# yanqinJiang/Animate3D

Measured on AMD Instinct MI355X. Metric: UNet denoise-steps/sec, 4view×16frame×512² MV-VDM @1/2/4/8 GPU, higher is better.
Workload: dtype bf16; 1 GPU; BASELINE config 2: 4 views x 16 frames x 512^2 px (64x64 latent), CFG-doubled batch V=8 videos, one MVUNetMotionModel.forward per step, SD1.5 MV-VDM UNet 1.53 B params, seeded synthetic weights; parallelism=single GPU

## Files before the change

animate3d_amd/csrc/gemm_common.h:

```cpp
#pragma once
#include "common.h"

struct GemmParams {
  const uint16_t* X; int64_t ldx;
  const uint16_t* W; int64_t ldw;
  const float* bias;
  const uint16_t* rowbias; int64_t rb_div;
  const uint16_t* R; int64_t ldr;
  uint16_t* Y; int64_t ldy;
  int64_t M, N, K;
  float alpha, beta;
  int vec16;
  int out_f32;
  int abl;
  int B, H, Wd, Cin, Ho, Wo, stride, up, He, We;
  int64_t tiles_n, tiles_m;
  int ksplit, nk_item;
  float* ws; int64_t ws_bytes;
  const uint16_t* X2; int64_t ldx2; int64_t K1;
  int direct;
};

constexpr int EPI_LINEAR = 0, EPI_GEGLU = 1;

static inline int a3d_gemm_kernel_of(int flags) { return flags & A3D_GEMM_KERNEL_MASK; }
static inline int a3d_gemm_reserved_cus_of(int flags) { return flags & A3D_GEMM_RESERVED_CUS_MASK; }

A3D_DEV float epi_scale(float v, float alpha) { return __fmul_rn(v, alpha); }
A3D_DEV float epi_axpy(float v, float beta, float r) { return __fmaf_rn(beta, r, v); }

A3D_DEV float gelu_erf(float gte) {
  const float x = fabsf(gte) * 0.70710678118654752f;
  const float t = __builtin_amdgcn_rcpf(fmaf(0.3275911f, x, 1.0f));
  float poly = fmaf(1.061405429f, t, -1.453152027f);
  poly = fmaf(poly, t, 1.421413741f);
  poly = fmaf(poly, t, -0.284496736f);
  poly = fmaf(poly, t, 0.254829592f);
  poly *= t;
  const float e = __builtin_amdgcn_exp2f(-x * x * 1.4426950408889634f);
  const float erfx = fmaf(-poly, e, 1.0f);
  const float hg = __fmul_rn(0.5f, gte);
  return __fmaf_rn(fabsf(hg), erfx, hg);
}

A3D_DEV f32x2_t splat2(float v) { return f32x2_t{v, v}; }
A3D_DEV f32x2_t gelu_erf2(f32x2_t g) {
  const f32x2_t x = __builtin_elementwise_abs(g) * 0.70710678118654752f;
  const f32x2_t den = __builtin_elementwise_fma(splat2(0.3275911f), x, splat2(1.0f));
  const f32x2_t t = {__builtin_amdgcn_rcpf(den[0]), __builtin_amdgcn_rcpf(den[1])};
  f32x2_t poly = __builtin_elementwise_fma(splat2(1.061405429f), t, splat2(-1.453152027f));
  poly = __builtin_elementwise_fma(poly, t, splat2(1.421413741f));
  poly = __builtin_elementwise_fma(poly, t, splat2(-0.284496736f));
  poly = __builtin_elementwise_fma(poly, t, splat2(0.254829592f));
  poly = poly * t;
  const f32x2_t a = (-x) * x * 1.4426950408889634f;
  const f32x2_t e = {__builtin_amdgcn_exp2f(a[0]), __builtin_amdgcn_exp2f(a[1])};
  const f32x2_t erfx = __builtin_elementwise_fma(-poly, e, splat2(1.0f));
  const f32x2_t hg = g * 0.5f;
  return __builtin_elementwise_fma(__builtin_elementwise_abs(hg), erfx, hg);
}
A3D_DEV void geglu8(const float (&hv)[8], const float (&gv)[8], const float (&bh)[8], const float (&bg)[8], float (&y)[8]) {
#pragma unroll
  for (int e = 0; e < 4; ++e) {
    const f32x2_t gg = f32x2_t{gv[2 * e], gv[2 * e + 1]} + f32x2_t{bg[2 * e], bg[2 * e + 1]};
    const f32x2_t hh = f32x2_t{hv[2 * e], hv[2 * e + 1]} + f32x2_t{bh[2 * e], bh[2 * e + 1]};
    const f32x2_t yy = hh * gelu_erf2(gg);
    y[2 * e] = yy[0]; y[2 * e + 1] = yy[1];
  }
}

static __device__ u32x4_t g_zero_page[4];

A3D_DEV uint32_t lds_addr(const void* p) {
  return (uint32_t)(uintptr_t)(__attribute__((address_space(3))) const void*)p;
}
A3D_DEV void glds16_v(const void* gsrc, uint32_t lds_dst) {
  unsigned keep;
  asm volatile("s_mov_b32 %0, m0\n\ts_mov_b32 m0, %2\n\ts_nop 0\n\tglobal_load_lds_dwordx4 %1, off\n\ts_mov_b32 m0, %0"
               : "=&s"(keep) : "v"(gsrc), "s"(__builtin_amdgcn_readfirstlane(lds_dst)) : "memory");
}
A3D_DEV void glds16_s(uint32_t voff, const void* sbase, uint32_t lds_dst) {
  unsigned keep;
  asm volatile("s_mov_b32 %0, m0\n\ts_mov_b32 m0, %3\n\ts_nop 0\n\tglobal_load_lds_dwordx4 %1, %2\n\ts_mov_b32 m0, %0"
               : "=&s"(keep) : "v"(voff), "s"(sbase), "s"(__builtin_amdgcn_readfirstlane(lds_dst)) : "memory");
}
A3D_DEV const uint16_t* scalar_ptr(const uint16_t* ptr) {
  const uint64_t a = (uint64_t)(uintptr_t)ptr;
  return (const uint16_t*)(uintptr_t)(((uint64_t)(uint32_t)__builtin_amdgcn_readfirstlane((int)(a >> 32)) << 32) |
                                      (uint32_t)__builtin_amdgcn_readfirstlane((int)(uint32_t)a));
}
A3D_DEV u32x4_t lds_vload128(const void* p) {
  return *(const volatile __attribute__((address_space(3))) u32x4_t*)(uintptr_t)lds_addr(p);
}
A3D_DEV u32x2_t lds_vload64(const void* p) {
  return *(const volatile __attribute__((address_space(3))) u32x2_t*)(uintptr_t)lds_addr(p);
}
A3D_DEV void wave_lds_fence() {
  __builtin_amdgcn_fence(__ATOMIC_RELEASE, "wavefront");
  __builtin_amdgcn_wave_barrier();
  __builtin_amdgcn_fence(__ATOMIC_ACQUIRE, "wavefront");
}

template <int EPI, int NB, bool RES>
A3D_DEV void persist_epilogue(const GemmParams& p, f32x16_t (&acc)[NB][2], float* const stg, const float* const bias_lds,
                              const uint16_t* const rowbias_lds, const int64_t m0, const int64_t n0, const int wm, const int wblk,
                              const int wblk_last, const int lane) {
  const int l31 = lane & 31, g = lane >> 5;
  constexpr int SROW = 68;
  constexpr int NP = (NB + 1) / 2;
  u32x4_t rres[RES ? 2 : 1][RES ? 4 : 1];
  auto pass_cols = [&](int ps) { return (2 * ps + 1 < NB) ? 64 : 32; };
  auto pass_col0 = [&](int ps) { return ((2 * ps + 1 < NB) ? wblk + 2 * ps : wblk_last) * 32; };
  auto load_res = [&](int pi, int slot) {
    if constexpr (RES) {
      const int tm = pi / NP, ps = pi % NP;
      const int64_t mbase = m0 + wm * 64 + tm * 32;
      const int64_t nbase = n0 + pass_col0(ps);
      if (pass_cols(ps) == 64) {
#pragma unroll
        for (int j = 0; j < 4; ++j) {
          const int64_t m = mbase + 8 * j + (lane >> 3);
          rres[slot][j] = *reinterpret_cast<const u32x4_t*>(p.R + m * p.ldr + nbase + 8 * (lane & 7));
        }
      } else {
#pragma unroll
        for (int j = 0; j < 2; ++j) {
          const int64_t m = mbase + 16 * j + (lane >> 2);
          rres[slot][j] = *reinterpret_cast<const u32x4_t*>(p.R + m * p.ldr + nbase + 8 * (lane & 3));
        }
      }
    }
  };
  if constexpr (RES) load_res(0, 0);
  if constexpr (EPI == EPI_GEGLU || !RES) {
    constexpr int RS = (EPI == EPI_GEGLU) ? 64 : 128;
    char* const stg16 = reinterpret_cast<char*>(stg);
    const int wsw = (EPI == EPI_GEGLU) ? ((l31 >> 1) & 3) : (l31 & 7);
    const int whalf = 8 * (g ^ ((l31 >> 3) & 1));
    auto unswap = [](u32x4_t o, int row) {
      const bool sw = row & 8;
      u32x4_t r;
      r[0] = sw ? o[2] : o[0]; r[1] = sw ? o[3] : o[1]; r[2] = sw ? o[0] : o[2]; r[3] = sw ? o[1] : o[3];
      return r;
    };
    constexpr int BUF2 = 32 * RS;
#pragma unroll
    for (int pi = 0; pi < 2 * NP; ++pi) {
      const int tm = pi / NP, ps = pi % NP;
      const int ncol = pass_cols(ps);
      const int64_t mbase = m0 + wm * 64 + tm * 32;
      const int64_t nbase = n0 + pass_col0(ps);
      char* const sb = stg16 + (pi & 1) * BUF2;
      if constexpr (EPI == EPI_GEGLU) {
        u32x4_t bq[2][4];
        auto fetch = [&](int q2, int slot) __attribute__((always_inline)) {
#pragma unroll
          for (int h = 0; h < 2; ++h) {
            const int c0 = 8 * (2 * q2 + h) + 4 * g;
            bq[slot][2 * h] = lds_vload128(bias_lds + pass_col0(ps) + c0);
            bq[slot][2 * h + 1] = lds_vload128(bias_lds + pass_col0(ps) + 32 + c0);
          }
        };
        fetch(0, 0);
#pragma unroll
        for (int q2 = 0; q2 < 2; ++q2) {
          if (q2 + 1 < 2) fetch(q2 + 1, (q2 + 1) & 1);
          __builtin_amdgcn_sched_barrier(0);
          float hv[8], gv[8], bh[8], bg[8], y[8];
#pragma unroll
          for (int h = 0; h < 2; ++h) {
            const u32x4_t b0 = bq[q2 & 1][2 * h], b1 = bq[q2 & 1][2 * h + 1];
#pragma unroll
            for (int j = 0; j < 4; ++j) { bh[4 * h + j] = __uint_as_float(b0[j]); bg[4 * h + j] = __uint_as_float(b1[j]); }
#pragma unroll
            for (int j = 0; j < 4; ++j) { hv[4 * h + j] = acc[2 * ps][tm][4 * (2 * q2 + h) + j]; gv[4 * h + j] = acc[2 * ps + 1][tm][4 * (2 * q2 + h) + j]; }
          }
          geglu8(hv, gv, bh, bg, y);
#pragma unroll
          for (int h = 0; h < 2; ++h) {
            u32x2_t o;
            o[0] = pack16(y[4 * h], y[4 * h + 1]);
            o[1] = pack16(y[4 * h + 2], y[4 * h + 3]);
            *reinterpret_cast<u32x2_t*>(sb + l31 * RS + 16 * ((2 * q2 + h) ^ wsw) + whalf) = o;
          }
        }
        wave_lds_fence();
        const int cc = lane & 3;
        const int64_t oc = nbase / 2 + 8 * cc;
        u32x4_t ob[2];
#pragma unroll
        for (int j = 0; j < 2; ++j) {
          const int row = 16 * j + (lane >> 2);
          ob[j] = *reinterpret_cast<const u32x4_t*>(sb + row * RS + 16 * (cc ^ ((row >> 1) & 3)));
        }
#pragma unroll
        for (int j = 0; j < 2; ++j) {
          const int row = 16 * j + (lane >> 2);
          const int64_t m = mbase + row;
          const u32x4_t o = unswap(ob[j], row);
#ifdef A3D_ABLATIONS
          if (p.abl & 2) { asm volatile("" :: "v"(o[0]), "v"(o[1]), "v"(o[2]), "v"(o[3])); continue; }
          *reinterpret_cast<u32x4_t*>(p.Y + ((p.abl & 1) ? (m & 255) : m) * p.ldy + oc) = o;
#else
          *reinterpret_cast<u32x4_t*>(p.Y + m * p.ldy + oc) = o;
#endif
        }
      } else {
        constexpr int NQ = 8;
        const int nq = (2 * ps + 1 < NB) ? 8 : 4;
        u32x4_t bq[3];
        u32x2_t tq[3];
        auto fetch = [&](int idx, int slot) __attribute__((always_inline)) {
          const int c0 = (idx >> 2) * 32 + 8 * (idx & 3) + 4 * g;
          bq[slot] = lds_vload128(bias_lds + pass_col0(ps) + c0);
          tq[slot] = lds_vload64(rowbias_lds + pass_col0(ps) + c0);
        };
        auto quads = [&](auto with_c) __attribute__((always_inline)) {
          constexpr bool WITH = decltype(with_c)::value;
          if constexpr (WITH) { fetch(0, 0); fetch(1, 1); }
#pragma unroll
          for (int idx = 0; idx < NQ; ++idx) {
            if (idx >= nq) continue;
            const int tl = idx >> 2, q = idx & 3;
            const int tn = 2 * ps + tl;
            if constexpr (WITH) {
              if (idx + 2 < nq) fetch(idx + 2, (idx + 2) % 3);
              __builtin_amdgcn_sched_barrier(0);
            }
            float v[4] = {acc[tn][tm][4 * q], acc[tn][tm][4 * q + 1], acc[tn][tm][4 * q + 2], acc[tn][tm][4 * q + 3]};
            if constexpr (WITH) {
              const u32x4_t b = bq[idx % 3];
              v[0] += __uint_as_float(b[0]); v[1] += __uint_as_float(b[1]); v[2] += __uint_as_float(b[2]); v[3] += __uint_as_float(b[3]);
              const u32x2_t tb = tq[idx % 3];
              v[0] += lo16(tb[0]); v[1] += hi16(tb[0]); v[2] += lo16(tb[1]); v[3] += hi16(tb[1]);
            }
#pragma unroll
            for (int e = 0; e < 4; ++e) v[e] = epi_scale(v[e], p.alpha);
            u32x2_t o;
            o[0] = pack16(v[0], v[1]);
            o[1] = pack16(v[2], v[3]);
            *reinterpret_cast<u32x2_t*>(sb + l31 * RS + 16 * ((4 * tl + q) ^ wsw) + whalf) = o;
            if constexpr (WITH) __builtin_amdgcn_sched_barrier(0);
          }
        };
        if (p.bias || p.rowbias) quads(std::true_type{});
        else quads(std::false_type{});
        wave_lds_fence();
        const int lpr = ncol / 8;
        const int cc = lane & (lpr - 1);
        u32x4_t ob[4];
#pragma unroll
        for (int j = 0; j < 4; ++j) {
          if (j * (64 / lpr) >= 32) continue;
          const int row = (64 / lpr) * j + lane / lpr;
          ob[j] = *reinterpret_cast<const u32x4_t*>(sb + row * RS + 16 * (cc ^ (row & 7)));
        }
#pragma unroll
        for (int j = 0; j < 4; ++j) {
          if (j * (64 / lpr) >= 32) continue;
          const int row = (64 / lpr) * j + lane / lpr;
          const int64_t m = mbase + row;
          const u32x4_t o = unswap(ob[j], row);
#ifdef A3D_ABLATIONS
          if (p.abl & 2) { asm volatile("" :: "v"(o[0]), "v"(o[1]), "v"(o[2]), "v"(o[3])); continue; }
          *reinterpret_cast<u32x4_t*>(p.Y + ((p.abl & 1) ? (m & 255) : m) * p.ldy + nbase + 8 * cc) = o;
#else
          *reinterpret_cast<u32x4_t*>(p.Y + m * p.ldy + nbase + 8 * cc) = o;
#endif
        }
      }
    }
    return;
  }
#pragma unroll
  for (int pi = 0; pi < 2 * NP; ++pi) {
    const int tm = pi / NP, ps = pi % NP;
    const int ncol = pass_cols(ps);
    if constexpr (RES) { if (pi + 1 < 2 * NP) load_res(pi + 1, (pi + 1) & 1); }
#pragma unroll
    for (int tl = 0; tl < 2; ++tl) {
      const int tn = 2 * ps + tl;
      if (tn < NB) {
#pragma unroll
        for (int q = 0; q < 4; ++q) {
          float4 v;
          v.x = acc[tn][tm][4 * q]; v.y = acc[tn][tm][4 * q + 1]; v.z = acc[tn][tm][4 * q + 2]; v.w = acc[tn][tm][4 * q + 3];
          *reinterpret_cast<float4*>(stg + l31 * SROW + tl * 32 + 8 * q + 4 * g) = v;
        }
      }
    }
    wave_lds_fence();
    const int64_t mbase = m0 + wm * 64 + tm * 32;
    const int64_t nbase = n0 + pass_col0(ps);

    if constexpr (EPI == EPI_GEGLU) {
      const int cc = lane & 3;
      const int64_t oc = nbase / 2 + 8 * cc;
      float bh[8], bg[8];
      {
        const float* bl = bias_lds + (pass_col0(ps) + 8 * cc);
#pragma unroll
        for (int e = 0; e < 8; ++e) { bh[e] = bl[e]; bg[e] = bl[32 + e]; }
      }
#pragma unroll
      for (int j = 0; j < 2; ++j) {
        const int row = 16 * j + (lane >> 2);
        const int64_t m = mbase + row;
        const float4 h0 = *reinterpret_cast<const float4*>(stg + row * SROW + 8 * cc);
        const float4 h1 = *reinterpret_cast<const float4*>(stg + row * SROW + 8 * cc + 4);
        const float4 g0 = *reinterpret_cast<const float4*>(stg + row * SROW + 32 + 8 * cc);
        const float4 g1 = *reinterpret_cast<const float4*>(stg + row * SROW + 32 + 8 * cc + 4);
        const float hv[8] = {h0.x, h0.y, h0.z, h0.w, h1.x, h1.y, h1.z, h1.w};
        const float gv[8] = {g0.x, g0.y, g0.z, g0.w, g1.x, g1.y, g1.z, g1.w};
        float y[8];
        geglu8(hv, gv, bh, bg, y);
        u32x4_t o;
#pragma unroll
        for (int e = 0; e < 4; ++e) o[e] = pack16(y[2 * e], y[2 * e + 1]);
#ifdef A3D_ABLATIONS
        if (p.abl & 2) { asm volatile("" :: "v"(o[0]), "v"(o[1]), "v"(o[2]), "v"(o[3])); continue; }
        *reinterpret_cast<u32x4_t*>(p.Y + ((p.abl & 1) ? (m & 255) : m) * p.ldy + oc) = o;
#else
        *reinterpret_cast<u32x4_t*>(p.Y + m * p.ldy + oc) = o;
#endif
      }
    } else {
      const int lpr = ncol / 8;
      const int cc = lane & (lpr - 1);
      const int64_t n = nbase + 8 * cc;
      const int ncl = pass_col0(ps) + 8 * cc;
      float bv[8];
#pragma unroll
      for (int e = 0; e < 8; ++e) bv[e] = bias_lds[ncl + e];
      const u32x4_t tb = *reinterpret_cast<const u32x4_t*>(rowbias_lds + ncl);
#pragma unroll
      for (int j = 0; j < 4; ++j) {
        if (j * (64 / lpr) >= 32) continue;
        const int row = (64 / lpr) * j + lane / lpr;
        const int64_t m = mbase + row;
        const float4 a0 = *reinterpret_cast<const float4*>(stg + row * SROW + 8 * cc);
        const float4 a1 = *reinterpret_cast<const float4*>(stg + row * SROW + 8 * cc + 4);
        float v[8] = {a0.x, a0.y, a0.z, a0.w, a1.x, a1.y, a1.z, a1.w};
#pragma unroll
        for (int e = 0; e < 8; ++e) v[e] += bv[e];
#pragma unroll
        for (int e = 0; e < 4; ++e) { v[2 * e] += lo16(tb[e]); v[2 * e + 1] += hi16(tb[e]); }
#pragma unroll
        for (int e = 0; e < 8; ++e) v[e] = epi_scale(v[e], p.alpha);
        if constexpr (RES) {
          const u32x4_t tr = rres[pi & 1][j];
#pragma unroll
          for (int e = 0; e < 4; ++e) { v[2 * e] = epi_axpy(v[2 * e], p.beta, lo16(tr[e])); v[2 * e + 1] = epi_axpy(v[2 * e + 1], p.beta, hi16(tr[e])); }
        }
        u32x4_t o;
#pragma unroll
        for (int e = 0; e < 4; ++e) o[e] = pack16(v[2 * e], v[2 * e + 1]);
#ifdef A3D_ABLATIONS
        if (p.abl & 2) { asm volatile("" :: "v"(o[0]), "v"(o[1]), "v"(o[2]), "v"(o[3])); continue; }
        *reinterpret_cast<u32x4_t*>(p.Y + ((p.abl & 1) ? (m & 255) : m) * p.ldy + n) = o;
#else
        *reinterpret_cast<u32x4_t*>(p.Y + m * p.ldy + n) = o;
#endif
      }
    }
    wave_lds_fence();
  }
}

template <int NB, bool RES>
A3D_DEV void direct_epilogue(const GemmParams& p, f32x16_t (&acc)[NB][2], const float* const bias_lds, const uint16_t* const rowbias_lds,
                             const int64_t m0, const int64_t n0, const int wm, const int wblk, const int wblk_last, const int lane) {
  const int l31 = lane & 31, g = lane >> 5;
  const bool with = p.bias || p.rowbias;
#pragma unroll
  for (int tm = 0; tm < 2; ++tm) {
    const int64_t m = m0 + wm * 64 + tm * 32 + l31;
    uint16_t* const yrow = p.Y + m * p.ldy + n0;
    u32x4_t rr[RES ? NB : 1][2];
    if constexpr (RES) {
      const uint16_t* const rrow = p.R + m * p.ldr + n0;
#pragma unroll
      for (int tn = 0; tn < NB; ++tn) {
        const int col = (tn < NB - 1 ? wblk + tn : wblk_last) * 32 + 16 * g;
        rr[tn][0] = *reinterpret_cast<const u32x4_t*>(rrow + col);
        rr[tn][1] = *reinterpret_cast<const u32x4_t*>(rrow + col + 8);
      }
    }
#pragma unroll
    for (int tn = 0; tn < NB; ++tn) {
      const int col = (tn < NB - 1 ? wblk + tn : wblk_last) * 32 + 16 * g;
      float v[16];
#pragma unroll
      for (int r = 0; r < 16; ++r) v[r] = acc[tn][tm][r];
      if (with) {
#pragma unroll
        for (int q = 0; q < 4; ++q) {
          const u32x4_t b = lds_vload128(bias_lds + col + 4 * q);
#pragma unroll
          for (int e = 0; e < 4; ++e) v[4 * q + e] += __uint_as_float(b[e]);
        }
#pragma unroll
        for (int h = 0; h < 2; ++h) {
          const u32x4_t tb = lds_vload128(rowbias_lds + col + 8 * h);
#pragma unroll
          for (int e = 0; e < 4; ++e) { v[8 * h + 2 * e] += lo16(tb[e]); v[8 * h + 2 * e + 1] += hi16(tb[e]); }
        }
      }
#pragma unroll
      for (int r = 0; r < 16; ++r) v[r] = epi_scale(v[r], p.alpha);
      if constexpr (RES) {
#pragma unroll
        for (int h = 0; h < 2; ++h)
#pragma unroll
          for (int e = 0; e < 4; ++e) {
            v[8 * h + 2 * e] = epi_axpy(v[8 * h + 2 * e], p.beta, lo16(rr[tn][h][e]));
            v[8 * h + 2 * e + 1] = epi_axpy(v[8 * h + 2 * e + 1], p.beta, hi16(rr[tn][h][e]));
          }
      }
#pragma unroll
      for (int h = 0; h < 2; ++h) {
        u32x4_t o;
#pragma unroll
        for (int e = 0; e < 4; ++e) o[e] = pack16(v[8 * h + 2 * e], v[8 * h + 2 * e + 1]);
        *reinterpret_cast<u32x4_t*>(yrow + col + 8 * h) = o;
      }
    }
  }
}

__attribute__((visibility("hidden"))) int A3D_FN(a3d_launch_gemm_pp)(int conv, int epi, int nb, hipStream_t stream, const GemmParams& p, int cus);
__attribute__((visibility("hidden"))) int A3D_FN(a3d_launch_gemm_ring)(int nb, hipStream_t stream, const GemmParams& p, int cus);
```

animate3d_amd/csrc/gemm_conv.hip:

```cpp
#include "gemm_common.h"

namespace {

constexpr int BM = 128, BN = 128;
template <int BKT> struct TileCfg {
  static constexpr int LROW = BKT + 8;
  static constexpr int TILE_ELEMS = 128 * LROW;
  static constexpr int STAGE_BYTES = 2 * 2 * TILE_ELEMS * 2;
  static constexpr int EPI_BYTES = 4 * 32 * 68 * 4;
  static constexpr int SMEM_BYTES = STAGE_BYTES > EPI_BYTES ? STAGE_BYTES : EPI_BYTES;
  static constexpr int CPR = BKT / 8;
  static constexpr int RPT = 256 / CPR;
  static constexpr int NPASS = 128 / RPT;
};



template <int CONV, int EPI, int BKT, bool RES>
__global__ __launch_bounds__(256, (BKT == 64 ? 2 : 3)) void gemm_kernel(const GemmParams p) {
  using TC = TileCfg<BKT>;
  constexpr int LROW = TC::LROW, TILE_ELEMS = TC::TILE_ELEMS, NPASS = TC::NPASS, RPT = TC::RPT, BK = BKT;
  extern __shared__ __attribute__((aligned(16))) uint16_t smem[];
  const int tid = threadIdx.x;
  const int lane = tid & 63, wid = tid >> 6;
  const int wm = wid >> 1, wn = wid & 1;
  const int l31 = lane & 31, g = lane >> 5;

  const int64_t nblk = p.tiles_n * p.tiles_m;
  const int64_t lid = xcd_remap(blockIdx.x, nblk);
  const int64_t tile_n = lid % p.tiles_n, tile_m = lid / p.tiles_n;
  const int64_t m0 = tile_m * BM, n0 = tile_n * BN;

  const int kc = tid % TC::CPR;
  const int srow = tid / TC::CPR;

  const uint16_t* a_ptr[NPASS];
  int a_b[CONV == 2 ? NPASS : 1], a_y[CONV == 2 ? NPASS : 1], a_x[CONV == 2 ? NPASS : 1];
  bool a_ok[NPASS];
  int a_mask[NPASS];
#pragma unroll
  for (int i = 0; i < NPASS; ++i) {
    int64_t m = m0 + srow + RPT * i;
    a_ok[i] = m < p.M;
    if (m >= p.M) m = p.M - 1;
    if constexpr (CONV != 0) {
      const int hw = p.Ho * p.Wo;
      const int b = (int)(m / hw);
      const int rem = (int)(m - (int64_t)b * hw);
      const int oy = rem / p.Wo, ox = rem - oy * p.Wo;
      if constexpr (CONV == 2) {
        a_b[i] = b; a_y[i] = oy; a_x[i] = ox;
        a_ptr[i] = nullptr; a_mask[i] = 0;
      } else {
        const int y0 = oy * p.stride - 1, x0 = ox * p.stride - 1;
        a_ptr[i] = p.X + (((int64_t)b * p.H + y0) * p.Wd + x0) * p.Cin + kc * 8;
        int mask = 0;
#pragma unroll
        for (int t = 0; t < 9; ++t) {
          const int yy = y0 + t / 3, xx = x0 + t % 3;
          if (a_ok[i] && yy >= 0 && yy < p.H && xx >= 0 && xx < p.Wd) mask |= 1 << t;
        }
        a_mask[i] = mask;
      }
    } else {
      a_ptr[i] = p.X + m * p.ldx + kc * 8;
      a_mask[i] = 0;
    }
  }
  const uint16_t* w_ptr[NPASS];
#pragma unroll
  for (int i = 0; i < NPASS; ++i) {
    int64_t n = n0 + srow + RPT * i;
    if (n >= p.N) n = p.N - 1;
    w_ptr[i] = p.W + n * p.ldw + kc * 8;
  }

  struct RegTile { u32x4_t a[NPASS], w[NPASS]; };
  RegTile rt0, rt1;
  auto load_tile = [&](int64_t k0, RegTile& rt) {
    u32x4_t (&ra)[NPASS] = rt.a; u32x4_t (&rw)[NPASS] = rt.w;
    if constexpr (CONV != 0) {
      {
        const int kt64 = (int)(k0 >> 6);
        const int c64 = kt64 / 9, t = kt64 - 9 * c64;
        k0 = (int64_t)t * p.Cin + c64 * 64 + (k0 & 63);
      }
      const int tap = (int)(k0 / p.Cin);
      const int ci0 = (int)(k0 - (int64_t)tap * p.Cin);
      const int ky = tap / 3, kx = tap - ky * 3;
      if constexpr (CONV == 1) {
        const int64_t toff = ((int64_t)ky * p.Wd + kx) * p.Cin + ci0;
#pragma unroll
        for (int i = 0; i < NPASS; ++i) {
          if ((a_mask[i] >> tap) & 1) ra[i] = *reinterpret_cast<const u32x4_t*>(a_ptr[i] + toff);
          else ra[i] = u32x4_t{0u, 0u, 0u, 0u};
        }
      } else {
        const int He = p.He, We = p.We;
#pragma unroll
        for (int i = 0; i < NPASS; ++i) {
          const int yy = a_y[i] + ky - 1, xx = a_x[i] + kx - 1;
          const bool ok = a_ok[i] && yy >= 0 && yy < He && xx >= 0 && xx < We;
          if (ok) {
            const uint16_t* src = p.X + (((int64_t)a_b[i] * p.H + (yy >> 1)) * p.Wd + (xx >> 1)) * p.Cin + ci0 + kc * 8;
            ra[i] = *reinterpret_cast<const u32x4_t*>(src);
          } else {
            ra[i] = u32x4_t{0u, 0u, 0u, 0u};
          }
        }
      }
    } else {
#pragma unroll
      for (int i = 0; i < NPASS; ++i) ra[i] = *reinterpret_cast<const u32x4_t*>(a_ptr[i] + k0);
    }
#pragma unroll
    for (int i = 0; i < NPASS; ++i) rw[i] = *reinterpret_cast<const u32x4_t*>(w_ptr[i] + k0);
  };
  auto store_tile = [&](int buf, const RegTile& rt) {
    const u32x4_t (&ra)[NPASS] = rt.a; const u32x4_t (&rw)[NPASS] = rt.w;
    uint16_t* As = smem + (buf * 2 + 0) * TILE_ELEMS;
    uint16_t* Ws = smem + (buf * 2 + 1) * TILE_ELEMS;
#pragma unroll
    for (int i = 0; i < NPASS; ++i) {
      *reinterpret_cast<u32x4_t*>(As + (srow + RPT * i) * LROW + kc * 8) = ra[i];
      *reinterpret_cast<u32x4_t*>(Ws + (srow + RPT * i) * LROW + kc * 8) = rw[i];
    }
  };

  f32x16_t acc[2][2];
#pragma unroll
  for (int a = 0; a < 2; ++a)
#pragma unroll
    for (int b = 0; b < 2; ++b)
#pragma unroll
      for (int r = 0; r < 16; ++r) acc[a][b][r] = 0.f;

  u32x4_t rres[RES ? 4 : 1];
  const int ecc = lane & 7;
  const int64_t en = n0 + wn * 64 + 8 * ecc;
  const bool epf = RES && (EPI == EPI_LINEAR) && p.R != nullptr && p.vec16 && en + 8 <= p.N;
  auto prefetch_residual = [&](int tm) {
    if constexpr (RES) {
#pragma unroll
      for (int j = 0; j < 4; ++j) {
        int64_t m = m0 + wm * 64 + tm * 32 + 8 * j + (lane >> 3);
        if (m >= p.M) m = p.M - 1;
        rres[j] = *reinterpret_cast<const u32x4_t*>(p.R + m * p.ldr + en);
      }
    }
  };

  const int64_t nk = p.K / BK;
  auto compute = [&](int cur) {
    const uint16_t* As = smem + (cur * 2 + 0) * TILE_ELEMS;
    const uint16_t* Ws = smem + (cur * 2 + 1) * TILE_ELEMS;
    u32x4_t fw[2][2], fa[2][2];
    auto load_frags = [&](int slot, int ks) {
#pragma unroll
      for (int t = 0; t < 2; ++t) {
        fw[slot][t] = *reinterpret_cast<const u32x4_t*>(Ws + (wn * 64 + t * 32 + l31) * LROW + ks * 16 + g * 8);
        fa[slot][t] = *reinterpret_cast<const u32x4_t*>(As + (wm * 64 + t * 32 + l31) * LROW + ks * 16 + g * 8);
      }
    };
    load_frags(0, 0);
#pragma unroll
    for (int ks = 0; ks < BK / 16; ++ks) {
      if (ks + 1 < BK / 16) load_frags((ks + 1) & 1, ks + 1);
#pragma unroll
      for (int tn = 0; tn < 2; ++tn)
#pragma unroll
        for (int tm = 0; tm < 2; ++tm) acc[tn][tm] = mfma32(fw[ks & 1][tn], fa[ks & 1][tm], acc[tn][tm]);
    }
  };

  load_tile(0, rt0);
  store_tile(0, rt0);
  if (nk > 1) load_tile(1 * BK, rt0);
  if (nk > 2) load_tile(2 * BK, rt1);
  __syncthreads();
  for (int64_t kt = 0;;) {
    if (kt + 1 >= nk && epf) prefetch_residual(0);
    compute(0);
    if (kt + 1 < nk) store_tile(1, rt0);
    if (kt + 3 < nk) load_tile((kt + 3) * BK, rt0);
    __syncthreads();
    if (++kt >= nk) break;
    if (kt + 1 >= nk && epf) prefetch_residual(0);
    compute(1);
    if (kt + 1 < nk) store_tile(0, rt1);
    if (kt + 3 < nk) load_tile((kt + 3) * BK, rt1);
    __syncthreads();
    if (++kt >= nk) break;
  }

  constexpr int SROW = 68;
  float* const stg = reinterpret_cast<float*>(smem) + wid * (32 * SROW);
#pragma unroll
  for (int tm = 0; tm < 2; ++tm) {
  if (tm == 1) __syncthreads();
#pragma unroll
  for (int tn = 0; tn < 2; ++tn)
#pragma unroll
    for (int q = 0; q < 4; ++q) {
      float4 v;
      v.x = acc[tn][tm][4 * q]; v.y = acc[tn][tm][4 * q + 1]; v.z = acc[tn][tm][4 * q + 2]; v.w = acc[tn][tm][4 * q + 3];
      *reinterpret_cast<float4*>(stg + l31 * SROW + tn * 32 + 8 * q + 4 * g) = v;
    }
  __syncthreads();
  const int64_t mbase = m0 + wm * 64 + tm * 32;

  if constexpr (EPI == EPI_GEGLU) {
    const int cc = lane & 3;
    const int64_t nh = n0 + wn * 64 + 8 * cc;
    const int64_t oc = (n0 + wn * 64) / 2 + 8 * cc;
    if (nh + 32 < p.N + 0 && oc + 8 <= p.N / 2) {
      float bh[8], bg[8];
#pragma unroll
      for (int e = 0; e < 8; ++e) { bh[e] = p.bias ? p.bias[nh + e] : 0.f; bg[e] = p.bias ? p.bias[nh + 32 + e] : 0.f; }
#pragma unroll
      for (int j = 0; j < 2; ++j) {
        const int row = 16 * j + (lane >> 2);
        const int64_t m = mbase + row;
        if (m >= p.M) continue;
        const float4 h0 = *reinterpret_cast<const float4*>(stg + row * SROW + 8 * cc);
        const float4 h1 = *reinterpret_cast<const float4*>(stg + row * SROW + 8 * cc + 4);
        const float4 g0 = *reinterpret_cast<const float4*>(stg + row * SROW + 32 + 8 * cc);
        const float4 g1 = *reinterpret_cast<const float4*>(stg + row * SROW + 32 + 8 * cc + 4);
        const float hv[8] = {h0.x, h0.y, h0.z, h0.w, h1.x, h1.y, h1.z, h1.w};
        const float gv[8] = {g0.x, g0.y, g0.z, g0.w, g1.x, g1.y, g1.z, g1.w};
        float y[8];
        geglu8(hv, gv, bh, bg, y);
        u32x4_t o;
#pragma unroll
        for (int e = 0; e < 4; ++e) o[e] = pack16(y[2 * e], y[2 * e + 1]);
        *reinterpret_cast<u32x4_t*>(p.Y + m * p.ldy + oc) = o;
      }
    }
  } else {
    const int cc = lane & 7;
    const int64_t n = n0 + wn * 64 + 8 * cc;
    if (n < p.N) {
      const bool full = (n + 8 <= p.N) && p.vec16;
      float bv[8];
#pragma unroll
      for (int e = 0; e < 8; ++e) bv[e] = (p.bias && n + e < p.N) ? p.bias[n + e] : 0.f;
#pragma unroll
      for (int j = 0; j < 4; ++j) {
        const int row = 8 * j + (lane >> 3);
        const int64_t m = mbase + row;
        if (m >= p.M) continue;
        const float4 a0 = *reinterpret_cast<const float4*>(stg + row * SROW + 8 * cc);
        const float4 a1 = *reinterpret_cast<const float4*>(stg + row * SROW + 8 * cc + 4);
        float v[8] = {a0.x, a0.y, a0.z, a0.w, a1.x, a1.y, a1.z, a1.w};
#pragma unroll
        for (int e = 0; e < 8; ++e) v[e] += bv[e];
        const uint16_t* rb = p.rowbias ? p.rowbias + (m / p.rb_div) * p.N + n : nullptr;
        const uint16_t* rr = p.R ? p.R + m * p.ldr + n : nullptr;
        uint16_t* yy = p.Y + m * p.ldy + n;
        if (full) {
          if (rb) {
            const u32x4_t t = *reinterpret_cast<const u32x4_t*>(rb);
#pragma unroll
            for (int e = 0; e < 4; ++e) { v[2 * e] += lo16(t[e]); v[2 * e + 1] += hi16(t[e]); }
          }
#pragma unroll
          for (int e = 0; e < 8; ++e) v[e] = epi_scale(v[e], p.alpha);
          if constexpr (RES) {
            if (rr) {
              const u32x4_t t = rres[j];
#pragma unroll
              for (int e = 0; e < 4; ++e) { v[2 * e] = epi_axpy(v[2 * e], p.beta, lo16(t[e])); v[2 * e + 1] = epi_axpy(v[2 * e + 1], p.beta, hi16(t[e])); }
            }
          }
          if (p.out_f32) {
            float* yf = reinterpret_cast<float*>(p.Y) + m * p.ldy + n;
            *reinterpret_cast<float4*>(yf) = float4{v[0], v[1], v[2], v[3]};
            *reinterpret_cast<float4*>(yf + 4) = float4{v[4], v[5], v[6], v[7]};
          } else {
            u32x4_t o;
#pragma unroll
            for (int e = 0; e < 4; ++e) o[e] = pack16(v[2 * e], v[2 * e + 1]);
            *reinterpret_cast<u32x4_t*>(yy) = o;
          }
        } else {
#pragma unroll
          for (int hh = 0; hh < 2; ++hh) {
            if (n + 4 * hh + 4 > p.N) continue;
            float w[4] = {v[4 * hh], v[4 * hh + 1], v[4 * hh + 2], v[4 * hh + 3]};
            if (rb) {
              const u32x2_t t = *reinterpret_cast<const u32x2_t*>(rb + 4 * hh);
              w[0] += lo16(t[0]); w[1] += hi16(t[0]); w[2] += lo16(t[1]); w[3] += hi16(t[1]);
            }
#pragma unroll
            for (int e = 0; e < 4; ++e) w[e] = epi_scale(w[e], p.alpha);
            if (rr) {
              const u32x2_t t = *reinterpret_cast<const u32x2_t*>(rr + 4 * hh);
              w[0] = epi_axpy(w[0], p.beta, lo16(t[0])); w[1] = epi_axpy(w[1], p.beta, hi16(t[0]));
              w[2] = epi_axpy(w[2], p.beta, lo16(t[1])); w[3] = epi_axpy(w[3], p.beta, hi16(t[1]));
            }
            u32x2_t o;
            o[0] = pack16(w[0], w[1]);
            o[1] = pack16(w[2], w[3]);
            *reinterpret_cast<u32x2_t*>(yy + 4 * hh) = o;
          }
        }
      }
    }
  }
  if (tm == 0 && epf) prefetch_residual(1);
  }
}


constexpr int PBM = 256;
constexpr int PERSIST_MIN_FILL = 50;
struct PPPlan { int nb, S, cus; int64_t tiles_m, tiles_n; };
constexpr int SPLITK_MAX = 16;
#ifndef A3D_EXP_SPLITK_MINK
#define A3D_EXP_SPLITK_MINK 9
#endif
template <int CONV, int EPI>
bool plan_persist(const GemmParams& p, int flags, bool allow_split, PPPlan& out) {
  if (a3d_gemm_kernel_of(flags) == A3D_GEMM_TILE128 || p.out_f32) return false;
  static int cus_of[64] = {0};
  const int dev = a3d_current_device();
  if (cus_of[dev] == 0) {
    int n = 0;
    if (hipDeviceGetAttribute(&n, hipDeviceAttributeMultiprocessorCount, dev) != hipSuccess) return false;
    cus_of[dev] = n > 0 ? n : 256;
  }
  const int reserved = a3d_gemm_reserved_cus_of(flags);
  const int cus = cus_of[dev] - reserved > 32 ? cus_of[dev] - reserved : 32;
  if (!p.vec16 || p.K % 64 != 0 || p.M % PBM != 0 || (p.rowbias && p.rb_div % PBM != 0)) return false;
  if (p.ldw % 64 != 0 || (CONV == 0 && p.ldx % 64 != 0)) return false;
  if (CONV == 0 && (uint64_t)p.ldx * 16u >= (1ull << 31)) return false;
  if ((uint64_t)p.ldw * 16u >= (1ull << 31)) return false;
  if (CONV != 0 && ((uint64_t)p.B * p.H * p.Wd + 2u * p.Wd + 2u) * (uint64_t)p.Cin * 2u >= (1ull << 32)) return false;
  const int64_t tm = (p.M + PBM - 1) / PBM;
  const int nk = (int)(p.K / 64);
  const int unit = CONV ? 9 : 1;
  const int cus_plan = cus_of[dev];
  constexpr int OVH = 12;
  int64_t best = -1, best1 = -1;
  int bnb = 0, bS = 1, bnb1 = 0;
  for (int nb = 5; nb >= 4; --nb) {
    if (EPI == EPI_GEGLU && nb == 5) continue;
    if (p.N % (nb * 64) != 0) continue;
    const int64_t tiles = tm * (p.N / (nb * 64));
    for (int S = 1; S <= (allow_split && EPI == EPI_LINEAR ? SPLITK_MAX : 1); ++S) {
      if ((nk / unit) % S != 0 || (S > 1 && nk / S < A3D_EXP_SPLITK_MINK)) continue;
      const int64_t items = tiles * S;
      const int64_t rounds = (items + cus_plan - 1) / cus_plan;
      if (items * 100 < rounds * cus_plan * PERSIST_MIN_FILL) continue;
      if (S > 1 && p.ws != nullptr && items * nb * 65536 > p.ws_bytes) continue;
      const int64_t cost = rounds * (nk / S + OVH) * nb * (nb == 4 ? 108 : 100) + (S > 1 ? 100 * nb : 0);
      if (S == 1 && (best1 < 0 || cost < best1)) { best1 = cost; bnb1 = nb; }
      if (best < 0 || cost < best) { best = cost; bnb = nb; bS = S; }
    }
  }
  if (best < 0) return false;
  if (bS > 1 && best1 >= 0 && best * 100 > best1 * 85) { bnb = bnb1; bS = 1; }
  out.nb = bnb; out.S = bS; out.cus = cus;
  out.tiles_m = tm; out.tiles_n = p.N / (bnb * 64);
  return true;
}

struct RingPlan { int nb, cus, cus_plan; int64_t cost; };
#ifndef A3D_RING_VS_PP_PCT
#define A3D_RING_VS_PP_PCT 75
#endif
constexpr int RING_VS_PP_PCT = A3D_RING_VS_PP_PCT;
inline bool plan_ring(const GemmParams& p, int flags, RingPlan& out) {
  if (a3d_gemm_kernel_of(flags) == A3D_GEMM_TILE128 || a3d_gemm_kernel_of(flags) == A3D_GEMM_DIRECT || p.out_f32 || !p.vec16 || p.X2 != nullptr) return false;
  if (p.M % 128 != 0 || p.K % 64 != 0 || p.K < 256 || p.ldx % 64 != 0 || p.ldw % 64 != 0) return false;
  if ((uint64_t)p.ldx * 64u >= (1ull << 32) || (uint64_t)p.ldw * 256u >= (1ull << 32)) return false;
  if (p.rowbias && p.rb_div % 128 != 0) return false;
  int n = 0;
  if (hipDeviceGetAttribute(&n, hipDeviceAttributeMultiprocessorCount, a3d_current_device()) != hipSuccess || n <= 0) n = 256;
  const int reserved = a3d_gemm_reserved_cus_of(flags);
  out.cus_plan = n;
  out.cus = n - reserved > 32 ? n - reserved : 32;
  out.nb = 0; out.cost = 0;
  for (int nb : {5, 4, 2}) {
    if (p.N % (64 * nb) != 0) continue;
    const int64_t tiles = (p.M / 128) * (p.N / (64 * nb));
    const int64_t rounds = (tiles + out.cus - 1) / out.cus;
    const int64_t cost = rounds * (128 + 64 * nb);
    if (out.nb == 0 || cost < out.cost) { out.nb = nb; out.cost = cost; }
  }
  return out.nb != 0;
}

template <int CONV, int EPI>
int try_launch_persist(hipStream_t stream, GemmParams& p, int flags) {
  PPPlan pl;
  if (!plan_persist<CONV, EPI>(p, flags, p.ws != nullptr, pl)) return -1000;
  p.tiles_m = pl.tiles_m; p.tiles_n = pl.tiles_n;
  p.ksplit = pl.S; p.nk_item = (int)(p.K / 64) / pl.S;
  p.direct = (CONV == 0 && EPI == EPI_LINEAR && pl.S == 1 && p.X2 == nullptr && a3d_gemm_kernel_of(flags) == A3D_GEMM_DIRECT) ? 1 : 0;
  return A3D_FN(a3d_launch_gemm_pp)(CONV, EPI, pl.nb, stream, p, pl.cus);
}


template <int CONV, int EPI, int BKT, bool RES>
int launch_res(hipStream_t stream, GemmParams& p, int64_t nblk) {
  using TC = TileCfg<BKT>;
  static uint64_t attr_done = 0;
  if (int rc = a3d_once_per_device(attr_done, [] {
        return (int)hipFuncSetAttribute(reinterpret_cast<const void*>(&gemm_kernel<CONV, EPI, BKT, RES>),
                                        hipFuncAttributeMaxDynamicSharedMemorySize, TC::SMEM_BYTES); })) return rc;
  gemm_kernel<CONV, EPI, BKT, RES><<<dim3((unsigned)nblk), dim3(256), TC::SMEM_BYTES, stream>>>(p);
  return a3d_launch_status();
}

template <int CONV, int EPI, int BKT>
int launch_bk(hipStream_t stream, GemmParams& p, int64_t nblk) {
  if constexpr (EPI == EPI_LINEAR) {
    if (p.R != nullptr) return launch_res<CONV, EPI, BKT, true>(stream, p, nblk);
  }
  return launch_res<CONV, EPI, BKT, false>(stream, p, nblk);
}

template <int CONV, int EPI = EPI_LINEAR>
int launch(hipStream_t stream, GemmParams& p, int flags) {
  if (flags & ~(A3D_GEMM_RESERVED_CUS_MASK | A3D_GEMM_KERNEL_MASK)) return A3D_EINVAL;
  if (a3d_gemm_kernel_of(flags) > A3D_GEMM_DIRECT) return A3D_EINVAL;
  if constexpr (CONV == 0 && EPI == EPI_LINEAR) {
    RingPlan rp;
    if (plan_ring(p, flags, rp)) {
      PPPlan pl;
      bool ring = true;
      if (a3d_gemm_kernel_of(flags) != A3D_GEMM_RING && plan_persist<CONV, EPI>(p, flags, p.ws != nullptr, pl)) {
        const int64_t tiles = pl.tiles_m * pl.tiles_n * pl.S;
        const int64_t pp_cost = ((tiles + rp.cus_plan - 1) / rp.cus_plan) * (256 + 64 * pl.nb) * RING_VS_PP_PCT;
        ring = pl.S == 1 && rp.cost * 100 < pp_cost;
      }
      if (ring) {
        p.tiles_m = p.M / 128; p.tiles_n = p.N / (64 * rp.nb);
        return A3D_FN(a3d_launch_gemm_ring)(rp.nb, stream, p, rp.cus);
      }
    }
  }
  {
    const int rc = try_launch_persist<CONV, EPI>(stream, p, flags);
    if (rc != -1000) return rc;
  }
  p.tiles_m = (p.M + BM - 1) / BM;
  p.tiles_n = (p.N + BN - 1) / BN;
  const int64_t nblk = p.tiles_m * p.tiles_n;
  if (nblk <= 0 || nblk > 0x7fffffffLL) return A3D_EINVAL;
  const bool small = (CONV == 0 && p.K <= 640) || nblk < 768;
  if (small) return launch_bk<CONV, EPI, 32>(stream, p, nblk);
  return launch_bk<CONV, EPI, 64>(stream, p, nblk);
}

inline bool aligned16(const void* p) { return (reinterpret_cast<uintptr_t>(p) & 15u) == 0; }

}

namespace {
template <int CONV>
int64_t splitk_ws_bytes(const GemmParams& p, int flags) {
  PPPlan pl;
  GemmParams q = p;
  q.ws = nullptr; q.ws_bytes = 0;
  if (flags & ~(A3D_GEMM_RESERVED_CUS_MASK | A3D_GEMM_KERNEL_MASK)) return 0;
  if (!plan_persist<CONV, EPI_LINEAR>(q, flags, true, pl) || pl.S <= 1) return 0;
  return pl.tiles_m * pl.tiles_n * pl.S * pl.nb * 65536;
}
}

static int gemm_entry(a3d_stream_t stream, const void* X, int64_t ldx, const void* W, int64_t ldw,
                      const float* bias, const void* rowbias, int64_t rb_div, const void* R, int64_t ldr,
                      void* Y, int64_t ldy, int64_t M, int64_t N, int64_t K, float alpha, float beta, int flags,
                      void* ws, int64_t ws_bytes, int64_t* ws_needed) {
  if (!X || !W || !Y || M <= 0 || N <= 0 || K <= 0) return A3D_EINVAL;
  if (K % 64 != 0 || N % 4 != 0) return A3D_EINVAL;
  if (ldx % 8 != 0 || ldw % 8 != 0 || ldy % 4 != 0 || (R && ldr % 4 != 0)) return A3D_EINVAL;
  if (!aligned16(X) || !aligned16(W) || (reinterpret_cast<uintptr_t>(Y) & 7u) || (R && (reinterpret_cast<uintptr_t>(R) & 7u)))
    return A3D_EINVAL;
  if (bias && (reinterpret_cast<uintptr_t>(bias) & 15u)) return A3D_EINVAL;
  if (rowbias && (rb_div <= 0 || (reinterpret_cast<uintptr_t>(rowbias) & 7u))) return A3D_EINVAL;
  GemmParams p{};
  p.X = (const uint16_t*)X; p.ldx = ldx; p.W = (const uint16_t*)W; p.ldw = ldw;
  p.bias = bias; p.rowbias = (const uint16_t*)rowbias; p.rb_div = rowbias ? rb_div : 1;
  p.R = (const uint16_t*)R; p.ldr = ldr; p.Y = (uint16_t*)Y; p.ldy = ldy;
  p.M = M; p.N = N; p.K = K; p.alpha = alpha; p.beta = beta;
  p.vec16 = (ldy % 8 == 0) && aligned16(Y) && (!R || (ldr % 8 == 0 && aligned16(R))) && (!rowbias || (N % 8 == 0 && aligned16(rowbias)));
  if (ws_needed) { *ws_needed = splitk_ws_bytes<0>(p, flags); return 0; }
  if (ws && ws_bytes > 0 && aligned16(ws)) { p.ws = (float*)ws; p.ws_bytes = ws_bytes; }
  return launch<0>((hipStream_t)stream, p, flags);
}

extern "C" int A3D_FN(a3d_gemm)(a3d_stream_t stream, const void* X, int64_t ldx, const void* W, int64_t ldw,
                             const float* bias, const void* rowbias, int64_t rb_div, const void* R, int64_t ldr,
                             void* Y, int64_t ldy, int64_t M, int64_t N, int64_t K, float alpha, float beta, int flags) {
  return gemm_entry(stream, X, ldx, W, ldw, bias, rowbias, rb_div, R, ldr, Y, ldy, M, N, K, alpha, beta, flags, nullptr, 0, nullptr);
}

extern "C" int A3D_FN(a3d_gemm_ws)(a3d_stream_t stream, const void* X, int64_t ldx, const void* W, int64_t ldw,
                                const float* bias, const void* rowbias, int64_t rb_div, const void* R, int64_t ldr,
                                void* Y, int64_t ldy, int64_t M, int64_t N, int64_t K, float alpha, float beta, int flags,
                                void* ws, int64_t ws_bytes, int64_t* ws_needed) {
  return gemm_entry(stream, X, ldx, W, ldw, bias, rowbias, rb_div, R, ldr, Y, ldy, M, N, K, alpha, beta, flags, ws, ws_bytes, ws_needed);
}

extern "C" int A3D_FN(a3d_gemm2)(a3d_stream_t stream, const void* X, int64_t ldx, const void* X2, int64_t ldx2, int64_t K1,
                              const void* W, int64_t ldw, const float* bias, void* Y, int64_t ldy, int64_t M, int64_t N, int64_t K, int flags) {
  if (!X || !X2 || !W || !Y || M <= 0 || N <= 0 || K <= 0 || K1 <= 0 || K1 >= K) return A3D_EINVAL;
  if (K % 64 != 0 || K1 % 64 != 0 || N % 8 != 0) return A3D_EINVAL;
  if (ldx % 8 != 0 || ldx2 % 8 != 0 || ldw % 8 != 0 || ldy % 8 != 0) return A3D_EINVAL;
  if (!aligned16(X) || !aligned16(X2) || !aligned16(W) || !aligned16(Y)) return A3D_EINVAL;
  if (bias && (reinterpret_cast<uintptr_t>(bias) & 15u)) return A3D_EINVAL;
  if (flags & ~(A3D_GEMM_RESERVED_CUS_MASK | A3D_GEMM_KERNEL_MASK)) return A3D_EINVAL;
  if (ldx2 % 64 != 0 || (uint64_t)ldx2 * 16u >= (1ull << 31)) return A3D_EUNSUPPORTED;
  GemmParams p{};
  p.X = (const uint16_t*)X; p.ldx = ldx; p.X2 = (const uint16_t*)X2; p.ldx2 = ldx2; p.K1 = K1;
  p.W = (const uint16_t*)W; p.ldw = ldw; p.bias = bias; p.rb_div = 1; p.Y = (uint16_t*)Y; p.ldy = ldy;
  p.M = M; p.N = N; p.K = K; p.alpha = 1.f; p.beta = 0.f; p.vec16 = 1;
  const int rc = try_launch_persist<0, EPI_LINEAR>((hipStream_t)stream, p, flags);
  return rc == -1000 ? A3D_EUNSUPPORTED : rc;
}

extern "C" int A3D_FN(a3d_gemm_f32out)(a3d_stream_t stream, const void* X, int64_t ldx, const void* W, int64_t ldw,
                                    const float* bias, float* Y, int64_t ldy, int64_t M, int64_t N, int64_t K, float alpha) {
  if (!X || !W || !Y || M <= 0 || N <= 0 || K <= 0) return A3D_EINVAL;
  if (K % 64 != 0 || N % 8 != 0 || ldx % 8 != 0 || ldw % 8 != 0 || ldy % 4 != 0) return A3D_EINVAL;
  if (!aligned16(X) || !aligned16(W) || !aligned16(Y)) return A3D_EINVAL;
  if (bias && (reinterpret_cast<uintptr_t>(bias) & 15u)) return A3D_EINVAL;
  GemmParams p{};
  p.X = (const uint16_t*)X; p.ldx = ldx; p.W = (const uint16_t*)W; p.ldw = ldw;
  p.bias = bias; p.rb_div = 1; p.Y = (uint16_t*)Y; p.ldy = ldy;
  p.M = M; p.N = N; p.K = K; p.alpha = alpha; p.beta = 0.f; p.vec16 = 1; p.out_f32 = 1;
  return launch<0>((hipStream_t)stream, p, 0);
}

static int conv_entry(a3d_stream_t stream, const void* X, const void* Wp, const float* bias,
                      const void* rowbias, int64_t rb_div, const void* R, void* Y,
                      int B, int H, int W, int Cin, int Cout, int stride, int up2x, int flags,
                      void* ws, int64_t ws_bytes, int64_t* ws_needed) {
  if (!X || !Wp || !Y || B <= 0 || H <= 0 || W <= 0) return A3D_EINVAL;
  if (Cin % 64 != 0 || Cout % 4 != 0 || (stride != 1 && stride != 2)) return A3D_EINVAL;
  if (up2x < 0 || up2x > 7 || (up2x > 1 && !(up2x & 1)) || (up2x && stride != 1)) return A3D_EINVAL;
  if (!aligned16(X) || !aligned16(Wp) || (reinterpret_cast<uintptr_t>(Y) & 7u)) return A3D_EINVAL;
  if (bias && (reinterpret_cast<uintptr_t>(bias) & 15u)) return A3D_EINVAL;
  if (rowbias && rb_div <= 0) return A3D_EINVAL;
  const int He = up2x ? 2 * H - ((up2x >> 1) & 1) : H, We = up2x ? 2 * W - ((up2x >> 2) & 1) : W;
  if (He <= 0 || We <= 0) return A3D_EINVAL;
  GemmParams p{};
  p.X = (const uint16_t*)X; p.ldx = Cin; p.W = (const uint16_t*)Wp; p.ldw = (int64_t)9 * Cin;
  p.bias = bias; p.rowbias = (const uint16_t*)rowbias; p.rb_div = rowbias ? rb_div : 1;
  p.R = (const uint16_t*)R; p.ldr = Cout; p.Y = (uint16_t*)Y; p.ldy = Cout;
  p.B = B; p.H = H; p.Wd = W; p.Cin = Cin; p.stride = stride; p.up = up2x ? 1 : 0; p.He = He; p.We = We;
  p.Ho = (He + 2 - 3) / stride + 1; p.Wo = (We + 2 - 3) / stride + 1;
  p.M = (int64_t)B * p.Ho * p.Wo; p.N = Cout; p.K = (int64_t)9 * Cin;
  p.alpha = 1.f; p.beta = 1.f;
  p.vec16 = (Cout % 8 == 0) && aligned16(Y) && (!R || aligned16(R)) && (!rowbias || aligned16(rowbias));
  if (ws_needed) { *ws_needed = up2x ? splitk_ws_bytes<2>(p, flags) : splitk_ws_bytes<1>(p, flags); return 0; }
  if (ws && ws_bytes > 0 && aligned16(ws)) { p.ws = (float*)ws; p.ws_bytes = ws_bytes; }
  return up2x ? launch<2>((hipStream_t)stream, p, flags) : launch<1>((hipStream_t)stream, p, flags);
}

extern "C" int A3D_FN(a3d_conv3x3)(a3d_stream_t stream, const void* X, const void* Wp, const float* bias,
                                const void* rowbias, int64_t rb_div, const void* R, void* Y,
                                int B, int H, int W, int Cin, int Cout, int stride, int up2x, int flags) {
  return conv_entry(stream, X, Wp, bias, rowbias, rb_div, R, Y, B, H, W, Cin, Cout, stride, up2x, flags, nullptr, 0, nullptr);
}

extern "C" int A3D_FN(a3d_conv3x3_ws)(a3d_stream_t stream, const void* X, const void* Wp, const float* bias,
                                   const void* rowbias, int64_t rb_div, const void* R, void* Y,
                                   int B, int H, int W, int Cin, int Cout, int stride, int up2x, int flags,
                                   void* ws, int64_t ws_bytes, int64_t* ws_needed) {
  return conv_entry(stream, X, Wp, bias, rowbias, rb_div, R, Y, B, H, W, Cin, Cout, stride, up2x, flags, ws, ws_bytes, ws_needed);
}

extern "C" int A3D_FN(a3d_gemm_geglu)(a3d_stream_t stream, const void* X, int64_t ldx, const void* W, int64_t ldw,
                                   const float* bias, void* Y, int64_t ldy, int64_t M, int64_t N2, int64_t K, int flags) {
  if (!X || !W || !Y || M <= 0 || N2 <= 0 || K <= 0) return A3D_EINVAL;
  if (K % 64 != 0 || N2 % 64 != 0 || ldx % 8 != 0 || ldw % 8 != 0 || ldy % 8 != 0) return A3D_EINVAL;
  if (!aligned16(X) || !aligned16(W) || !aligned16(Y)) return A3D_EINVAL;
  GemmParams p{};
  p.X = (const uint16_t*)X; p.ldx = ldx; p.W = (const uint16_t*)W; p.ldw = ldw;
  p.bias = bias; p.rb_div = 1; p.Y = (uint16_t*)Y; p.ldy = ldy;
  p.M = M; p.N = N2; p.K = K; p.alpha = 1.f; p.beta = 0.f; p.vec16 = 1;
  return launch<0, EPI_GEGLU>((hipStream_t)stream, p, flags);
}
```

Baseline: 2.373 denoise-steps/s.

## Add specialized 3x3 conv kernel for tiny output-channel counts

```diff
diff --git a/animate3d_amd/csrc/conv_small.hip b/animate3d_amd/csrc/conv_small.hip
--- /dev/null
+++ b/animate3d_amd/csrc/conv_small.hip
@@ -0,0 +1,142 @@
+#include "gemm_common.h"
+
+namespace {
+
+constexpr int CS_NCH = 12;
+constexpr int CS_NT = 6;
+constexpr int CS_MAX_PIX = 32 * CS_NCH;
+constexpr int CS_PIX = 72;
+
+__global__ __launch_bounds__(256, 2) void conv3x3_small_cout_kernel(const GemmParams p, const int R, const int strips) {
+  extern __shared__ __attribute__((aligned(16))) uint16_t smem[];
+  const int tid = threadIdx.x;
+  const int lane = tid & 63, wid = tid >> 6;
+  const int l15 = lane & 15, kg = lane >> 4;
+  const int H = p.H, W = p.Wd, Cin = p.Cin, Cout = (int)p.N;
+  const int WP = W + 2;
+  const uint32_t lid = xcd_remap32(blockIdx.x, gridDim.x);
+  const int b = (int)(lid / (uint32_t)strips);
+  const int y0 = (int)(lid % (uint32_t)strips) * R;
+  const int rows = R < H - y0 ? R : H - y0;
+
+  const int nchunk = (R + 2) * W * 8;
+  const int64_t xbase = (((int64_t)b * H + y0 - 1) * W) * Cin;
+  const int soff0 = (tid >> 3) * Cin + (tid & 7) * 8;
+  int sdst[CS_NCH];
+  uint32_t sload = 0;
+#pragma unroll
+  for (int i = 0; i < CS_NCH; ++i) {
+    const int c = tid + 256 * i;
+    const int pix = c >> 3, kc = c & 7;
+    const int r = pix / W, x = pix - r * W;
+    const int y = y0 - 1 + r;
+    sdst[i] = c < nchunk ? (r * WP + x + 1) * CS_PIX + kc * 8 : -1;
+    if (c < nchunk && y >= 0 && y < H) sload |= 1u << i;
+  }
+  u32x4_t rin[CS_NCH];
+  auto load_in = [&](int s) {
+#pragma unroll
+    for (int i = 0; i < CS_NCH; ++i) {
+      if ((sload >> i) & 1u) rin[i] = *reinterpret_cast<const u32x4_t*>(p.X + (xbase + soff0 + 32 * i * Cin + s * 64));
+      else rin[i] = u32x4_t{0u, 0u, 0u, 0u};
+    }
+  };
+  auto store_in = [&]() {
+#pragma unroll
+    for (int i = 0; i < CS_NCH; ++i)
+      if (sdst[i] >= 0) *reinterpret_cast<u32x4_t*>(smem + sdst[i]) = rin[i];
+  };
+  auto load_w = [&](int s, u32x4_t (&w)[9][2]) {
+#pragma unroll
+    for (int t = 0; t < 9; ++t)
+#pragma unroll
+      for (int ks = 0; ks < 2; ++ks) {
+        if (l15 < Cout) w[t][ks] = *reinterpret_cast<const u32x4_t*>(p.W + (int64_t)l15 * p.ldw + t * Cin + s * 64 + ks * 32 + kg * 8);
+        else w[t][ks] = u32x4_t{0u, 0u, 0u, 0u};
+      }
+  };
+  const int npix = rows * W;
+  const int ntiles = (npix + 15) >> 4;
+  int taddr[CS_NT];
+#pragma unroll
+  for (int ti = 0; ti < CS_NT; ++ti) {
+    int pix = (wid + 4 * ti) * 16 + l15;
+    pix = pix < npix ? pix : npix - 1;
+    const int y = pix / W, x = pix - y * W;
+    taddr[ti] = (y * WP + x) * CS_PIX + kg * 8;
+  }
+  f32x4_t acc[CS_NT];
+#pragma unroll
+  for (int ti = 0; ti < CS_NT; ++ti) acc[ti] = f32x4_t{0.f, 0.f, 0.f, 0.f};
+
+  u32x4_t wf[9][2];
+  load_in(0);
+  load_w(0, wf);
+  for (int idx = tid; idx < (R + 2) * 16; idx += 256) {
+    const int r = idx >> 4, side = (idx >> 3) & 1, kc = idx & 7;
+    *reinterpret_cast<u32x4_t*>(smem + (r * WP + (side ? W + 1 : 0)) * CS_PIX + kc * 8) = u32x4_t{0u, 0u, 0u, 0u};
+  }
+  const int ns = Cin >> 6;
+  for (int s = 0; s < ns; ++s) {
+    if (s) __syncthreads();
+    store_in();
+    if (s + 1 < ns) load_in(s + 1);
+    __syncthreads();
+#pragma unroll
+    for (int ti = 0; ti < CS_NT; ++ti) {
+      if (wid + 4 * ti >= ntiles) continue;
+#pragma unroll
+      for (int t = 0; t < 9; ++t)
+#pragma unroll
+        for (int ks = 0; ks < 2; ++ks) {
+          const u32x4_t bf = *reinterpret_cast<const u32x4_t*>(smem + taddr[ti] + ((t / 3) * WP + (t % 3)) * CS_PIX + ks * 32);
+          acc[ti] = mfma16(wf[t][ks], bf, acc[ti]);
+        }
+    }
+    if (s + 1 < ns) load_w(s + 1, wf);
+  }
+
+  const int co = 4 * kg;
+  if (co >= Cout) return;
+  float bv[4];
+#pragma unroll
+  for (int e = 0; e < 4; ++e) bv[e] = p.bias ? p.bias[co + e] : 0.f;
+#pragma unroll
+  for (int ti = 0; ti < CS_NT; ++ti) {
+    const int pix = (wid + 4 * ti) * 16 + l15;
+    if (pix >= npix) continue;
+    const int64_t m = ((int64_t)b * H + y0) * W + pix;
+    float v[4];
+#pragma unroll
+    for (int e = 0; e < 4; ++e) v[e] = acc[ti][e] + bv[e];
+    if (p.rowbias) {
+      const u32x2_t t = *reinterpret_cast<const u32x2_t*>(p.rowbias + (m / p.rb_div) * Cout + co);
+      v[0] += lo16(t[0]); v[1] += hi16(t[0]); v[2] += lo16(t[1]); v[3] += hi16(t[1]);
+    }
+#pragma unroll
+    for (int e = 0; e < 4; ++e) v[e] = epi_scale(v[e], p.alpha);
+    u32x2_t o;
+    o[0] = pack16(v[0], v[1]);
+    o[1] = pack16(v[2], v[3]);
+    *reinterpret_cast<u32x2_t*>(p.Y + m * p.ldy + co) = o;
+  }
+}
+
+}
+
+int A3D_FN(a3d_launch_conv_small)(hipStream_t s, const GemmParams& p) {
+  if (p.N > 16 || p.N % 4 != 0 || p.stride != 1 || p.up || p.R || p.out_f32 || p.Cin % 64 != 0) return A3D_EUNSUPPORTED;
+  if (p.rowbias && (reinterpret_cast<uintptr_t>(p.rowbias) & 7u)) return A3D_EUNSUPPORTED;
+  int R = CS_MAX_PIX / p.Wd - 2;
+  if (R > 30) R = 30;
+  if (R < 1) return A3D_EUNSUPPORTED;
+  if (R > p.H) R = p.H;
+  const int strips = (p.H + R - 1) / R;
+  R = (p.H + strips - 1) / strips;
+  const int64_t grid = (int64_t)p.B * strips;
+  if (grid > 0x7fffffffLL || (int64_t)CS_MAX_PIX * p.Cin > 0x3fffffffLL) return A3D_EUNSUPPORTED;
+  const size_t lds = (size_t)(R + 2) * (p.Wd + 2) * CS_PIX * sizeof(uint16_t);
+  if (lds > 65536) return A3D_EUNSUPPORTED;
+  conv3x3_small_cout_kernel<<<dim3((unsigned)grid), dim3(256), lds, s>>>(p, R, strips);
+  return a3d_launch_status();
+}
diff --git a/animate3d_amd/csrc/gemm_common.h b/animate3d_amd/csrc/gemm_common.h
--- a/animate3d_amd/csrc/gemm_common.h
+++ b/animate3d_amd/csrc/gemm_common.h
@@ -430,3 +430,4 @@
 
 __attribute__((visibility("hidden"))) int A3D_FN(a3d_launch_gemm_pp)(int conv, int epi, int nb, hipStream_t stream, const GemmParams& p, int cus);
 __attribute__((visibility("hidden"))) int A3D_FN(a3d_launch_gemm_ring)(int nb, hipStream_t stream, const GemmParams& p, int cus);
+__attribute__((visibility("hidden"))) int A3D_FN(a3d_launch_conv_small)(hipStream_t stream, const GemmParams& p);
diff --git a/animate3d_amd/csrc/gemm_conv.hip b/animate3d_amd/csrc/gemm_conv.hip
--- a/animate3d_amd/csrc/gemm_conv.hip
+++ b/animate3d_amd/csrc/gemm_conv.hip
@@ -558,6 +558,10 @@
   p.vec16 = (Cout % 8 == 0) && aligned16(Y) && (!R || aligned16(R)) && (!rowbias || aligned16(rowbias));
   if (ws_needed) { *ws_needed = up2x ? splitk_ws_bytes<2>(p, flags) : splitk_ws_bytes<1>(p, flags); return 0; }
   if (ws && ws_bytes > 0 && aligned16(ws)) { p.ws = (float*)ws; p.ws_bytes = ws_bytes; }
+  if (Cout <= 16 && stride == 1 && !up2x && !R && (flags & ~A3D_GEMM_RESERVED_CUS_MASK) == 0) {
+    const int rc = A3D_FN(a3d_launch_conv_small)((hipStream_t)stream, p);
+    if (rc != A3D_EUNSUPPORTED) return rc;
+  }
   return up2x ? launch<2>((hipStream_t)stream, p, flags) : launch<1>((hipStream_t)stream, p, flags);
 }
 
```

After: 2.374 denoise-steps/s, median of 2. About the same (+0.1%).
